# Q-Minh/point-cloud-processing

Measured on AMD Instinct MI355X. Metric: kNN+normal-estimation Mqueries/s (k=15), higher is better.
Workload: dtype f32

## Files before the change

### point-cloud-processing_amd/csrc/pcpx_api.hip

```cpp
#include "pcpx_internal.h"
#include "pcpx_radius.h"
#include "pcpx_features.h"

#include <algorithm>
#include <cstring>
#include <functional>
#include <vector>

namespace pcpx {
namespace {

struct Slice {
    u64 lo, hi, gf, gc;
};
Slice slice_of(const Index& ix, u64 sorted_first, u64 sorted_count)
{
    const u64 n = ix.n;
    Slice s;
    s.lo = sorted_first < n ? sorted_first : n;
    s.hi = sorted_count > n - s.lo ? n : s.lo + sorted_count;
    s.gf = s.lo / GROUP;
    const u64 gend = (s.hi + GROUP - 1) / GROUP;
    s.gc = gend > s.gf ? gend - s.gf : 0;
    return s;
// ... 878 lines not shown
    PCPX_HIP(hipMemcpy(dp.p, xyz, m * 3 * sizeof(float), hipMemcpyHostToDevice));
    if ((st = launch_normal_single(dp.as<float>(), m, dn.as<float>(), nullptr)) != PCPX_OK) return st;
    PCPX_HIP(hipMemcpy(out_normal, dn.p, 3 * sizeof(float), hipMemcpyDeviceToHost));
    return PCPX_OK;
    });
}

int pcpx_estimate_normals_batch(const float* xyz, const uint64_t* offsets, uint64_t nrows, int device, float* out_normals)
{
    return on_shared(device, "pcpx_estimate_normals_batch", [&](DeviceShared& shared) -> int {
    int st;
    if (nrows == 0) return PCPX_OK;
    if (!offsets || !out_normals) return PCPX_ERR_INVALID;
    for (u64 r = 0; r < nrows; ++r)
        if (offsets[r + 1] < offsets[r]) {
            set_error("pcpx_estimate_normals_batch: offsets must not decrease (row %llu)", static_cast<unsigned long long>(r));
            return PCPX_ERR_INVALID;
        }
    const u64 total = offsets[nrows] - offsets[0];
    if (total > 0 && !xyz) return PCPX_ERR_INVALID;
    DevBuf dp(shared.pool), doff(shared.pool), dn(shared.pool);
    if ((st = dp.alloc(total * 3 * sizeof(float))) != PCPX_OK || (st = doff.alloc((nrows + 1) * sizeof(u64))) != PCPX_OK ||
        (st = dn.alloc(nrows * 3 * sizeof(float))) != PCPX_OK)
        return st;
    if (total > 0) PCPX_HIP(hipMemcpyAsync(dp.p, xyz + 3 * offsets[0], total * 3 * sizeof(float), hipMemcpyHostToDevice, nullptr));
    PCPX_HIP(hipMemcpyAsync(doff.p, offsets, (nrows + 1) * sizeof(u64), hipMemcpyHostToDevice, nullptr));
    if ((st = launch_normals_csr(dp.as<float>(), doff.as<u64>(), nrows, dn.as<float>(), nullptr)) != PCPX_OK) return st;
    PCPX_HIP(hipMemcpyAsync(out_normals, dn.p, nrows * 3 * sizeof(float), hipMemcpyDeviceToHost, nullptr));
    PCPX_HIP(hipStreamSynchronize(nullptr));
    return PCPX_OK;
    });
}

int pcpx_debug_eps_test_mode(pcpx_index* h, int mode)
{
    return on_index(h, "pcpx_debug_eps_test_mode", ANY_INDEX, [&](Index* ix) -> int {
    if (mode < 0 || mode > 2) {
        set_error("pcpx_debug_eps_test_mode: mode is 0 (automatic), 1 (in the compaction) or 2 (per candidate)");
        return PCPX_ERR_INVALID;
    }
    ix->eps_test_mode = mode;
    return PCPX_OK;
    });
}

int pcpx_debug_set(pcpx_index* h, const char* name, int64_t value)
{
    return on_index(h, "pcpx_debug_set", ANY_INDEX, [&](Index* ix) -> int {
    if (!name) return PCPX_ERR_INVALID;
    const std::string key(name);
    if (key == "long_groups_first") {
        ix->tuning.lpt = value != 0;
        ix->sched.state = 0;
    } else if (key == "gather_outputs") {
        ix->tuning.gather = value != 0;
    } else if (key == "gather_counts") {
        ix->tuning.gather_counts = value != 0;
    } else {
        set_error("pcpx_debug_set: no setting called '%s'", name);
        return PCPX_ERR_INVALID;
    }
    return PCPX_OK;
    });
}

int pcpx_debug_get(pcpx_index* h, const char* name, int64_t* out_value)
{
    return on_index(h, "pcpx_debug_get", ANY_INDEX, [&](Index* ix) -> int {
    if (!name || !out_value) return PCPX_ERR_INVALID;
    const std::string key(name);
    if (key == "build_redos") {
        *out_value = ix->build_redos;
    } else if (key == "full_buckets") {
        int64_t c = 0;
        for (u32 w = 0; w < 8; ++w) c += __builtin_popcount(ix->full_buckets[w]);
        *out_value = c;
    } else if (key == "schedule_state") {
        *out_value = ix->sched.state;
    } else {
        set_error("pcpx_debug_get: no figure called '%s'", name);
        return PCPX_ERR_INVALID;
    }
    return PCPX_OK;
    });
}

int pcpx_debug_group_times(pcpx_index* h, uint32_t* out_ticks, uint64_t capacity, uint64_t* out_groups)
{
    return on_index(h, "pcpx_debug_group_times", ANY_INDEX, [&](Index* ix) -> int {
    if (!out_groups) return PCPX_ERR_INVALID;
    *out_groups = ix->sched.state ? ix->sched.gc : 0;
    if (*out_groups == 0) return PCPX_OK;
    if (!out_ticks || capacity < *out_groups) return PCPX_ERR_CAPACITY;
    PCPX_HIP(hipMemcpyAsync(out_ticks, ix->sched.d_gtime, *out_groups * sizeof(u32), hipMemcpyDeviceToHost, ix->stream));
    PCPX_HIP(hipStreamSynchronize(ix->stream));
    return PCPX_OK;
    });
}

int pcpx_knn_group_costs_dev(pcpx_index* h, uint32_t k, float eps, uint32_t group_stride, uint32_t* d_out_events, uint64_t capacity,
                             uint64_t* out_samples)
{
    return on_index(h, "pcpx_knn_group_costs_dev", ANY_INDEX, [&](Index* ix) -> int {
    if (!out_samples || group_stride == 0) return PCPX_ERR_INVALID;
    if (ix->shard.on) return shard_unsupported(*ix, "pcpx_knn_group_costs_dev");
    const u64 groups = (ix->n + GROUP - 1) / GROUP;
// ... 367 lines not shown
```

### point-cloud-processing_amd/csrc/pcpx_device.h

```cpp
#ifndef PCPX_DEVICE_H
#define PCPX_DEVICE_H

#include "pcpx_internal.h"

#include <cmath>
#include <limits>
#include <type_traits>

#pragma clang fp contract(off)

namespace pcpx {
namespace {

constexpr int WAVES_PER_BLOCK = 1;

__device__ __forceinline__ u32 wave_in_block() { return __builtin_amdgcn_readfirstlane(threadIdx.x >> 6); }

__device__ __forceinline__ u32 virtual_block()
{
    u32 per = gridDim.x >> 3;
    return (blockIdx.x & 7u) * per + (blockIdx.x >> 3);
}

__device__ __forceinline__ float sq3(float dx, float dy, float dz) { return dx * dx + dy * dy + dz * dz; }
// ... 25 lines not shown
    NodeBox4 out;
    u32* o = reinterpret_cast<u32*>(&out);
#pragma unroll
    for (int i = 0; i < 16; ++i) {
        o[i] = a[i];
        o[16 + i] = b[i];
    }
    return out;
}

__device__ __forceinline__ bool any_lane(bool c) { return __builtin_amdgcn_ballot_w64(c) != 0ull; }

template <class T>
__device__ __forceinline__ T load_const(const T* p)
{
    static_assert(sizeof(T) % 4 == 0, "record size");
    typedef const __attribute__((address_space(4))) u32* const_u32_ptr;
    const_u32_ptr c = (const_u32_ptr)(reinterpret_cast<uintptr_t>(p));
    T out;
    u32* o = reinterpret_cast<u32*>(&out);
#pragma unroll
    for (unsigned i = 0; i < sizeof(T) / 4; ++i) o[i] = c[i];
    return out;
}

__device__ __forceinline__ u32 lds_address(const void* p)
{
    return static_cast<u32>(reinterpret_cast<uintptr_t>(p));
}


template <bool X16, bool KEEP = false>
struct WalkerT {
    u64 pend;
    u32 ploc;
    int l;
    u64 leaf_need[W];

    static __device__ __forceinline__ u32 level_base(int d) { return 0x55555555u >> (32 - 2 * d); }

    template <class Need>
    __device__ __forceinline__ u32 child_mask(const TreeView& t, int d, u32 loc, Need&& need)
    {
        const u32 first_child = level_base(d + 1) + (loc << LOGW);
        const NodeBox4 cb = X16 ? load_node4(t.nodes + first_child) : load_const(reinterpret_cast<const NodeBox4*>(t.nodes + first_child));
        u32 m = 0;
#pragma unroll
        for (int c = W - 1; c >= 0; --c) {
            const u64 lanes = __builtin_amdgcn_ballot_w64(need(cb.c[c]));
            if (KEEP) leaf_need[c] = lanes;
            asm("s_cmp_lg_u64 %1, 0\n\ts_addc_u32 %0, %0, %0" : "+s"(m) : "s"(lanes) : "scc");
        }
        return m;
    }

    template <class Need>
    __device__ __forceinline__ bool start(const TreeView& t, Need&& need, u32& n_expand)
    {
        pend = 0;
        ploc = 0;
        l = 0;
        if (t.nleaves == 0) return false;
        const NodeBox root = load_const(t.nodes);
        if (!any_lane(need(root))) return false;
        if (t.depth == 0) return true;
        ++n_expand;
        l = t.depth - 1;
        pend = static_cast<u64>(child_mask(t, 0, 0u, need)) << (W * l);
        return false;
    }

    __device__ __forceinline__ bool done() const { return pend == 0; }
    __device__ __forceinline__ int pop(u32& loc)
    {
        int bit;
        asm("s_ff1_i32_b64 %0, %1\n\ts_bitset0_b64 %1, %0" : "=&s"(bit), "+s"(pend));
        const int h = bit >> LOGW;
        loc = ((ploc >> (LOGW * (h - l))) << LOGW) + (static_cast<u32>(bit) & (W - 1u));
        return h;
    }
    __device__ __forceinline__ void at_leaf(u32 loc)
    {
        ploc = loc >> LOGW;
        l = 0;
    }
    template <class Need>
    __device__ __forceinline__ void expand(const TreeView& t, int h, u32 loc, Need&& need)
    {
        l = h - 1;
        ploc = loc;
        pend |= static_cast<u64>(child_mask(t, t.depth - h, loc, need)) << (W * l);
    }

    template <class Need>
    __device__ __forceinline__ u32 leaves_of(const TreeView& t, u32 loc, Need&& need)
    {
        l = 0;
        ploc = loc;
        return child_mask(t, t.depth - 1, loc, need);
    }

    template <class Need>
    __device__ __forceinline__ bool next(const TreeView& t, Need&& need, u32& leaf, u32& n_expand)
    {
        while (pend != 0) {
            const int bit = __builtin_ctzll(pend);
// ... 76 lines not shown
```

### point-cloud-processing_amd/csrc/pcpx_internal.h

```cpp
#ifndef PCPX_INTERNAL_H
#define PCPX_INTERNAL_H

#include <cstring>
#include <hip/hip_runtime.h>

#include <cstdint>
#include <mutex>
#include <new>
#include <string>
#include <vector>

#include "pcpx.h"

namespace pcpx {

using u32 = std::uint32_t;
using u64 = std::uint64_t;

constexpr int LEAF = 8;
constexpr int LOGW = 2;
constexpr int W = 1 << LOGW;
constexpr int GROUP = 64;
constexpr int LEAVES_PER_GROUP = GROUP / LEAF;
constexpr int MAXDEPTH = 15;
// ... 118 lines not shown
    int idx_bits = 1;
    int sorted_from_bit = 24;
    const u64* finish_words = nullptr;
    const u32* finish_first_pass = nullptr;
    u32 full_buckets[8] = {0, 0, 0, 0, 0, 0, 0, 0};
    u32 build_redos = 0;
    u32 low_pass_tiles = ~0u;
    void* d_sort_tmp = nullptr;
    size_t sort_tmp_bytes = 0;
    Leaf* d_leaves = nullptr;
    NodeBox* d_nodes = nullptr;
    u64 nodes_cap = 0;
    u32* d_scalars = nullptr;
    u32 nleaves = 0;
    int depth = 0;
    u32 leaf0 = 0;

    struct Interval {
        int family;
        hipEvent_t a, b;
    };
    bool profiling = false;
    std::vector<Interval> intervals;

    u32* d_queue = nullptr;
    u32 queue_set = 0;
    u32* queue_now = nullptr;
    u32* queue_clear = nullptr;
    u64* d_multi = nullptr;
    size_t multi_bytes = 0;

    void* d_scratch = nullptr;
    size_t scratch_bytes = 0;

    hipStream_t copy_stream = nullptr;
    DevPool pool;
    PinnedStage pinned;
    u32 few_epoch = 0;
    struct Sched {
        u32* d_gtime = nullptr;
        u32* d_order = nullptr;
        u64 cap = 0;
        u64 gf = 0, gc = 0;
        int kcap = 0;
        u32 k = 0;
        int state = 0;
    } sched;
    float4* d_nc4 = nullptr;
    u32* d_pos_of = nullptr;
    u64 nc4_cap = 0, pos_of_cap = 0;
    bool pos_of_valid = false;
    struct Tuning {
        int lpt = 1;
        int gather_counts = 0;
        int gather = 0;
    } tuning;
    int eps_test_mode = 0;

    struct Shard {
        bool on = false;
        u32 rank = 0, world = 1;
        u64 n_glob = 0;
        u64 g_first = 0, g_count = 0;
        u64 core_g0 = 0;
        u64 core_l0 = 0;
        u64 core_count = 0;
        u32 halo_cells = 0;
        u32 k_hint = 0;
        bool explicit_range = false;
        u64 range_first = 0, range_count = 0;
        bool everything = false;
        bool borrowed = false;
        const float* cloud = nullptr;
        u32* d_sel = nullptr;
        u32* d_need = nullptr;
        u32* d_grid = nullptr;
        u32* d_hist12 = nullptr;
        u32* d_plan = nullptr;
        u32* d_big = nullptr;
        u32* d_tile_cnt = nullptr;
        u64 tile_cap = 0;
        u64* d_words = nullptr;
        float* d_tau = nullptr;
        u32* d_fail = nullptr;
        u64 cap_loc = 0;
        u32 verified_k = 0;
        float verified_eps = -1.f;
        u64 verified_first = 0, verified_count = 0;
        u64 last_failed = 0, total_failed = 0, enlargements = 0;
    } shard;

    const u64* sorted_codes() const { return finish_words ? finish_words : d_codes[1]; }
    u32* perm() const { return d_perm; }
    TreeView view() const { return TreeView{d_leaves, d_nodes, nleaves, static_cast<u32>(n), depth, leaf0}; }
};

struct ProfileScope {
    Index& ix;
    int family;
    hipEvent_t a = nullptr, b = nullptr;
    ProfileScope(Index& i, int fam) : ix(i), family(fam)
    {
        if (!ix.profiling) return;
        if (hipEventCreate(&a) != hipSuccess || hipEventCreate(&b) != hipSuccess) {
            a = b = nullptr;
            return;
// ... 297 lines not shown
```

### point-cloud-processing_amd/csrc/pcpx_query.hip

```cpp
#include "pcpx_device.h"
#include "pcpx_eig3.h"

namespace pcpx {

namespace {

constexpr size_t STATS_EXTRA = 16 + 5 * 65536 - 8;
constexpr u64 PAD_KEY = 0x7F800000FFFFFFFFull;

__device__ __forceinline__ u64 pad_key_here()
{
    u32 lo = static_cast<u32>(PAD_KEY), hi = static_cast<u32>(PAD_KEY >> 32);
    asm volatile("" : "+v"(lo), "+v"(hi));
    return (static_cast<u64>(hi) << 32) | lo;
}

__device__ __forceinline__ void ce(u64& a, u64& b)
{
    double x = __longlong_as_double(static_cast<long long>(a)), y = __longlong_as_double(static_cast<long long>(b));
    double lo, hi;
    asm("v_min_f64 %0, %1, %2" : "=v"(lo) : "v"(x), "v"(y));
    asm("v_max_f64 %0, %1, %2" : "=v"(hi) : "v"(x), "v"(y));
    a = static_cast<u64>(__double_as_longlong(lo));
    b = static_cast<u64>(__double_as_longlong(hi));
// ... 279 lines not shown
                 "v_add_u32_e32 %[pos], 1, %[pos]"
                 : [wa] "+v"(wa), [pos] "+v"(pos)
                 : [d2] "v"(d2), [tau] "v"(tau), [lo] "s"(lo), [sv] "s"(saved)
                 : "vcc", "memory");
}

__device__ __forceinline__ void append_if_shell(float d2, float tau, float lo, float dx, float dy, float dz, float eps, u32& pos,
                                                u32& wa, u64 saved)
{
    float m = fmaxf(fmaxf(fabsf(dx), fabsf(dy)), fabsf(dz));
    asm volatile("v_cmpx_le_f32_e32 %[d2], %[tau]\n\t"
                 "v_cmpx_lt_f32_e32 %[lo], %[d2]\n\t"
                 "v_cmpx_le_f32_e32 %[eps], %[m]\n\t"
                 "ds_write2_b32 %[wa], %[pos], %[d2] offset1:1\n\t"
                 "v_add_u32_e32 %[wa], 0x200, %[wa]\n\t"
                 "s_mov_b64 exec, %[sv]\n\t"
                 "v_add_u32_e32 %[pos], 1, %[pos]"
                 : [wa] "+v"(wa), [pos] "+v"(pos)
                 : [d2] "v"(d2), [tau] "v"(tau), [lo] "s"(lo), [m] "v"(m), [eps] "s"(eps), [sv] "s"(saved)
                 : "vcc", "memory");
}

constexpr int MINW8 = 8;
constexpr int MINW16 = 7;
constexpr int MINW32 = 4;
template <int KCAP>
constexpr float cap_mult() { return KCAP <= 8 ? 1.375f : KCAP <= 16 ? 1.25f : 1.125f; }
constexpr float CAP_GROW = 4.f;
template <int KCAP>
__device__ __forceinline__ float wave_radius_cap(float tau, bool valid, u32 lane)
{
    const float inf = std::numeric_limits<float>::infinity();
    asm volatile("" : "+v"(lane));
    const bool sample = (lane & 3u) == 1u;
    const float x = (valid && tau < inf) ? tau : inf;
    const u64 finite = __builtin_amdgcn_ballot_w64(sample && x < inf);
    const u32 nfinite = static_cast<u32>(__builtin_popcountll(finite));
    if (nfinite == 0) {
        const u64 any = __builtin_amdgcn_ballot_w64(x < inf);
        if (any == 0) return inf;
        return __uint_as_float(__builtin_amdgcn_readlane(__float_as_uint(x), static_cast<u32>(__builtin_ctzll(any)))) * cap_mult<KCAP>();
    }
    u32 rank = 0;
#pragma unroll
    for (u32 l = 1; l < 64; l += 4) {
        const float other = __uint_as_float(__builtin_amdgcn_readlane(__float_as_uint(x), l));
        rank += (other < x || (other == x && l < lane)) ? 1u : 0u;
    }
    const u64 is_med = __builtin_amdgcn_ballot_w64(sample && x < inf && rank == nfinite / 2);
    const float med = __uint_as_float(__builtin_amdgcn_readlane(__float_as_uint(x), static_cast<u32>(__builtin_ctzll(is_med))));
    return med * cap_mult<KCAP>();
}

struct MultiPass {
    const u64* lo = nullptr;
    u64* lo_out = nullptr;
    u64* keys = nullptr;
    u32 stride = 0;
    u32 offset = 0;
    u32 slot0 = 0;
};

struct KnnArgs {
    TreeView t;
    QueryView qv;
    u32 group_first, group_end, k;
    float eps, eps_thr;
    KnnOutputs o;
    MultiPass mp;
    u32* queue;
    unsigned long long* stats;
    KnnSchedule sch;
    u32* queue_clear;
};
typedef const __attribute__((address_space(4))) KnnArgs* knn_args_ptr;
__device__ __forceinline__ knn_args_ptr knn_args_here()
{
    u64 a = reinterpret_cast<u64>(__builtin_amdgcn_kernarg_segment_ptr());
    u32 lo = static_cast<u32>(a), hi = static_cast<u32>(a >> 32);
    asm volatile("" : "+s"(lo), "+s"(hi));
    return reinterpret_cast<knn_args_ptr>((static_cast<u64>(hi) << 32) | lo);
}
template <class T>
__device__ __forceinline__ T cold(const __attribute__((address_space(4))) T* field)
{
    static_assert(sizeof(T) % 4 == 0, "dwords");
    T out;
    u32* o = reinterpret_cast<u32*>(&out);
    const __attribute__((address_space(4))) u32* c = reinterpret_cast<const __attribute__((address_space(4))) u32*>(field);
#pragma unroll
    for (unsigned i = 0; i < sizeof(T) / 4; ++i) o[i] = c[i];
    return out;
}

template <int KCAP, bool SELF, int DIAG, bool MULTI, bool EPS_EACH, int NZ>
__device__ __forceinline__ void knn_group(const TreeView& tree, const u32 g, const float eps, const float eps_thr,
                                          unsigned long long* __restrict__ stats, u64* __restrict__ col, float* __restrict__ pub, const u32 lane,
                                          const u32 slot, const u32 part)
{
    constexpr bool STATS = DIAG == 1, COST = DIAG == 2;
    constexpr int BUF = buf_rows(KCAP);
    TreeView t = tree;
    asm volatile("" : "+s"(t.depth), "+s"(t.nodes));
    __builtin_amdgcn_s_setprio(PRIO_BASE);
    const knn_args_ptr ka = knn_args_here();
    const u32 k_arg = ka->k;
    const u32 pos_lo = ka->o.pos_lo, pos_hi = ka->o.pos_hi;
    MultiPass mp;
    if (MULTI) mp = cold(&ka->mp);
    const float* const known_d2 = STATS ? cold(&ka->o.d2) : nullptr;
    u32 k_here = k_arg;
    asm volatile("" : "+s"(k_here));
    const u32 k = k_here;
    u32 st_leaves = 0, st_expand = 0, st_compact = 0, st_app = 0, st_round2 = 0, st_seed_compact = 0, st_seed_app = 0, st_sparse = 0, st_owners = 0;
    u32 st_steps = 0;
    unsigned long long tc_walk = 0, tc_compact = 0, tc_leaf = 0, tc0 = 0, tc_mark = 0, tc_later_mark = 0;
    u32 st_later_lanes = 0;
    if (STATS) tc0 = __builtin_amdgcn_s_memtime();
    u32 tick0 = 0;
    if (!MULTI && DIAG == 0) tick0 = static_cast<u32>(__builtin_amdgcn_s_memtime());

    u32 p_here = g * GROUP + lane;
    asm volatile("" : "+v"(p_here));
    const u32 p = p_here;
    const u32 nq = SELF ? t.n : ka->qv.nq;
    const bool mine_of_part = ((p >> 3) & 7u) + 1u == part;
    const bool valid = p < nq && (!SELF || p - pos_lo < pos_hi - pos_lo) && (part == 0u || mine_of_part);
    float qx = 0.f, qy = 0.f, qz = 0.f;
    if (valid) {
        if (SELF) {
            const Leaf& lf = t.leaves[p / LEAF];
            qx = lf.x[p % LEAF];
            qy = lf.y[p % LEAF];
            qz = lf.z[p % LEAF];
        } else {
            qx = cold(&ka->qv.qx)[p];
            qy = cold(&ka->qv.qy)[p];
            qz = cold(&ka->qv.qz)[p];
        }
    }
    asm volatile("" : "+v"(qx), "+v"(qy), "+v"(qz));
    u64 lo_key = 0;
    bool has_lo = false;
    if (MULTI && mp.lo && valid) {
        lo_key = mp.lo[p - mp.slot0];
        has_lo = true;
    }
    u64 best[KCAP];
#pragma unroll
    for (int j = 0; j < KCAP; ++j) best[j] = (j < KCAP - static_cast<int>(k)) ? 0ull : PAD_KEY;
    const float inf = std::numeric_limits<float>::infinity();
    float tau = valid ? inf : -1.f;
    float tau_known = inf;
// ... 192 lines not shown
            u32 at, inside;
            if (packed_free > 0)
                asm volatile("v_cmpx_le_f32_e32 %[d2], %[tau]\n\t"
                             "v_mov_b32_e32 %[at], 0x200\n\t"
                             "ds_add_rtn_u32 %[at], %[slot], %[at]\n\t"
                             "s_waitcnt lgkmcnt(0)\n\t"
                             "v_subrev_u32_e32 %[m], %[end], %[at]\n\t"
                             "v_ashrrev_i32_e32 %[m], 31, %[m]\n\t"
                             "v_bfi_b32 %[at], %[m], %[at], %[spare]\n\t"
                             "ds_write2_b32 %[at], %[pos], %[d2] offset1:1\n\t"
                             "s_mov_b64 exec, %[saved]"
                             : [at] "=&v"(at), [m] "=&v"(inside)
                             : [d2] "v"(d2), [tau] "v"(q.w), [slot] "v"(slot), [end] "s"(wa_end), [spare] "s"(wa_end + 480u), [pos] "v"(posj), [saved] "s"(saved)
                             : "vcc", "memory");
            else
                asm volatile("v_cmpx_le_f32_e32 %[d2], %[tau]\n\t"
                             "v_mov_b32_e32 %[at], 0x200\n\t"
                             "ds_add_rtn_u32 %[at], %[slot], %[at]\n\t"
                             "s_waitcnt lgkmcnt(0)\n\t"
                             "ds_write2_b32 %[at], %[pos], %[d2] offset1:1\n\t"
                             "s_mov_b64 exec, %[saved]"
                             : [at] "=&v"(at)
                             : [d2] "v"(d2), [tau] "v"(q.w), [slot] "v"(slot), [pos] "v"(posj), [saved] "s"(saved)
                             : "vcc", "memory");
            s += 8u;
        } while (s < how_many);
        __builtin_amdgcn_wave_barrier();
        u32 now = wa;
        if (mine) {
            now = pub_wa[r];
            reinterpret_cast<float*>(pub_q + r)[3] = -1.f;
        }
        __builtin_amdgcn_wave_barrier();
        __builtin_amdgcn_s_setprio(PRIO_BASE);
        if (packed_free == 0) {
            wa = now;
            return 0ull;
        }
        const bool lost_keys = now > col_addr + (static_cast<u32>(BUF) << 9);
        wa = lost_keys ? wa : now;
        return __builtin_amdgcn_ballot_w64(lost_keys);
    };
    auto packed_take_back = [&](const u64 lost) {
        if (__builtin_amdgcn_inverse_ballot_w64(lost)) {
            const u32 column_end = col_addr + (static_cast<u32>(BUF) << 9);
            const u64 pad = pad_key_here();
            for (u32 a = wa; a < column_end; a += 512u) asm volatile("ds_write_b64 %0, %1" ::"v"(a), "v"(pad) : "memory");
        }
    };
    const u32 seed_count = s1 - s0;
    u32 packed_limit = packed_leaves ? PACKED_LEAVES : 0;
    for (u32 rounds = 0;;) {
        const u32 packed_limit_now = __builtin_amdgcn_readfirstlane(packed_limit);
        bool root_leaf = wk.start(t, need, st_expand);
        (void)root_leaf;
        if (STATS) tc_mark = __builtin_amdgcn_s_memtime();
        u32 direct = 0, direct_first = 0;
        for (;;) {
            if (direct == 0) {
                if (wk.done()) break;
                u32 node;
                const int h = wk.pop(node);
                ++st_expand;
                if (h > 1) {
                    wk.expand(t, h, node, need);
                } else {
                    direct_first = node << LOGW;
                    direct = wk.leaves_of(t, node, need);
                }
            }
            while (direct != 0) {
                u32 loc;
                {
                    u32 child;
                    asm("s_ff1_i32_b32 %0, %1\n\ts_bitset0_b32 %1, %0" : "=&s"(child), "+s"(direct));
                    loc = direct_first + child;
                }
                if (loc - s0 >= seed_count) {
                    if (STATS) tc_walk += __builtin_amdgcn_s_memtime() - tc_mark;
                    if (!packed_leaves) {
                        fold_if_needed(true, false);
                        candidates(loc, rounds != 0u);
                    } else {
                        const u32 c = loc & (W - 1u);
                        u64 who;
                        u32 how_many;
                        asm("s_cmp_eq_u32 %[c], 2\n\ts_cselect_b64 %[w], %[n2], %[n3]\n\t"
                            "s_cmp_eq_u32 %[c], 1\n\ts_cselect_b64 %[w], %[n1], %[w]\n\t"
                            "s_cmp_eq_u32 %[c], 0\n\ts_cselect_b64 %[w], %[n0], %[w]\n\t"
                            "s_bcnt1_i32_b64 %[m], %[w]"
                            : [w] "=&s"(who), [m] "=s"(how_many)
                            : [c] "s"(c), [n0] "s"(wk.leaf_need[0]), [n1] "s"(wk.leaf_need[1]), [n2] "s"(wk.leaf_need[2]), [n3] "s"(wk.leaf_need[3])
                            : "scc");
                        u32 packed_form, full_from;
                        asm("s_cmp_le_u32 %[m], %[lim]\n\ts_cselect_b32 %[pf], 1, 0\n\ts_cselect_b32 %[thr], %[tp], %[td]"
                            : [pf] "=&s"(packed_form), [thr] "=&s"(full_from)
                            : [m] "s"(how_many), [lim] "s"(packed_limit_now), [tp] "s"(wa_packed_full), [td] "s"(wa_full)
                            : "scc");
                        u64 todo = who;
                        for (;;) {
                            if ((__builtin_amdgcn_ballot_w64(wa >= full_from) & todo) != 0) fold(false);
                            if (packed_form == 0u) break;
                            if (STATS) tc_mark = __builtin_amdgcn_s_memtime();
                            todo = packed_leaf(loc, todo, how_many);
                            if (COST) st_steps += (how_many + 7u) >> 3;
                            if (STATS) {
                                asm volatile("" ::"v"(wa));
                                tc_leaf += __builtin_amdgcn_s_memtime() - tc_mark;
                            }
                            if (__builtin_expect(todo == 0, 1)) break;
                            packed_take_back(todo);
                            how_many = static_cast<u32>(__builtin_popcountll(todo));
                            full_from = 0u;
                        }
                        if (packed_form != 0u) {
                            if (COST) ++st_sparse;
                            if (STATS) ++st_leaves, ++st_sparse, st_owners += how_many;
// ... 103 lines not shown
        u32 id = t.leaves[ps / LEAF].id[ps % LEAF];
        asm volatile("" : "+v"(id));
        best[s] = real ? ((key & 0xFFFFFFFF00000000ull) | id) : key;
    }
    bool unordered = false;
#pragma unroll
    for (int s = 0; s + 1 < KCAP; ++s) unordered |= best[s] > best[s + 1];
    for (int round = 0; round < KCAP && any_lane(unordered); ++round) {
#pragma unroll
        for (int parity = 0; parity < 2; ++parity) {
#pragma unroll
            for (int s = parity; s + 1 < KCAP; s += 2) {
                const bool sw = best[s] > best[s + 1];
                const u64 a = sw ? best[s + 1] : best[s], b = sw ? best[s] : best[s + 1];
                best[s] = a;
                best[s + 1] = b;
                if (sw) {
                    const u32 pa = pos_slot(s), pb = pos_slot(s + 1);
                    pos_slot(s) = pb;
                    pos_slot(s + 1) = pa;
                }
            }
        }
        unordered = false;
#pragma unroll
        for (int s = 0; s + 1 < KCAP; ++s) unordered |= best[s] > best[s + 1];
    }
    auto restore_column = [&]() {
        const u64 pad = pad_key_here();
#pragma unroll
        for (int r = 0; r < (KCAP + 1) / 2; ++r) col[r * 64] = pad;
    };

    if (!valid) {
        restore_column();
        return;
    }
    u32 g_again = g;
    asm volatile("" : "+s"(g_again));
    u32 p_row = g_again * GROUP + lane;
    asm volatile("" : "+v"(p_row));
    const knn_args_ptr kb = knn_args_here();
    const KnnOutputs o = cold(&kb->o);
    u32 row = SELF ? t.leaves[p_row / LEAF].id[p_row % LEAF] : cold(&kb->qv.row)[p_row];
    if (SELF && o.by_position) row = p_row + o.pos_bias;
    if (SELF && o.tau) o.tau[p_row] = key_d2(best[KCAP - 1]);
    u32 found = 0;
    u32 okmask = 0;
    const u32 stride = o.row_stride ? o.row_stride : k;
    const u64 ob = static_cast<u64>(row) * stride;
    const bool whole_rows = stride == static_cast<u32>(KCAP) && first_slot == NZ && !STATS;
    auto store_whole_rows = [&](auto FS) {
        constexpr int fs = decltype(FS)::value;
#pragma unroll
        for (int c = 0; c < KCAP / 4; ++c) {
            u32 id4[4];
            float d4[4];
#pragma unroll
            for (int e = 0; e < 4; ++e) {
                const int sl = 4 * c + e + fs;
                const u64 key = sl < KCAP ? best[sl < KCAP ? sl : 0] : PAD_KEY;
                const bool ok = key != PAD_KEY;
                id4[e] = ok ? static_cast<u32>(key) : INVALID_ID;
                d4[e] = __uint_as_float(static_cast<u32>(key >> 32));
            }
            if (o.idx) *reinterpret_cast<uint4*>(o.idx + ob + 4 * c) = make_uint4(id4[0], id4[1], id4[2], id4[3]);
            if (o.d2) *reinterpret_cast<float4*>(o.d2 + ob + 4 * c) = make_float4(d4[0], d4[1], d4[2], d4[3]);
        }
    };
    if (whole_rows) store_whole_rows(std::integral_constant<int, NZ>{});
#pragma unroll
    for (int s = NZ; s < KCAP; ++s) {
        int j = s - first_slot;
        if (j >= 0) {
            u64 key = best[s];
            bool ok = key != PAD_KEY;
            if (!whole_rows) {
                if (o.idx) o.idx[ob + j] = ok ? static_cast<u32>(key) : INVALID_ID;
                if (o.d2 && !STATS) o.d2[ob + j] = __uint_as_float(static_cast<u32>(key >> 32));
            }
            found += ok ? 1u : 0u;
            okmask |= ok ? (1u << s) : 0u;
        }
    }
    if (!whole_rows) {
        for (u32 j = k; j < stride; ++j) {
            if (o.idx) o.idx[ob + j] = INVALID_ID;
            if (o.d2 && !STATS) o.d2[ob + j] = __uint_as_float(static_cast<u32>(PAD_KEY >> 32));
        }
    }
    if (o.cnt) o.cnt[row] = found;

    if (o.meandist) {
        float sum = 0.f;
#pragma unroll
        for (int s = NZ; s < KCAP; ++s) {
            bool ok = (okmask >> s) & 1u;
            float d = sqrtf(__uint_as_float(static_cast<u32>(best[s] >> 32)));
            sum += ok ? d : 0.f;
        }
        o.meandist[row] = sum / static_cast<float>(found);
    }

    if (o.normals || o.centroids || (SELF && o.nc4)) {
        float nbx[KCAP], nby[KCAP], nbz[KCAP];
#pragma unroll
        for (int s = NZ; s < KCAP; ++s) {
            const u32 ps = pos_slot(s);
            const Leaf& lf = t.leaves[ps / LEAF];
            nbx[s] = lf.x[ps % LEAF];
            nby[s] = lf.y[ps % LEAF];
            nbz[s] = lf.z[ps % LEAF];
        }
        float sx = 0.f, sy = 0.f, sz = 0.f;
#pragma unroll
        for (int s = NZ; s < KCAP; ++s) {
// ... 5 lines not shown
        float fn = static_cast<float>(found);
        float mx = sx / fn, my = sy / fn, mz = sz / fn;
        if (o.centroids) {
            o.centroids[3ull * row] = mx;
            o.centroids[3ull * row + 1] = my;
            o.centroids[3ull * row + 2] = mz;
        }
        if (!o.normals && !(SELF && o.nc4)) {
            restore_column();
            return;
        }
        float c00 = 0.f, c10 = 0.f, c11 = 0.f, c20 = 0.f, c21 = 0.f, c22 = 0.f;
#pragma unroll
        for (int s = NZ; s < KCAP; ++s) {
            bool ok = (okmask >> s) & 1u;
            float x = nbx[s], y = nby[s], z = nbz[s];
            float vx = ok ? x - mx : 0.f, vy = ok ? y - my : 0.f, vz = ok ? z - mz : 0.f;
            c00 += vx * vx;
            c10 += vy * vx;
            c11 += vy * vy;
            c20 += vz * vx;
            c21 += vz * vy;
            c22 += vz * vz;
        }
        float nrm[3], ev[3];
        eig3_smallest(c00, c10, c20, c11, c21, c22, nrm, ev);
        if (SELF && o.nc4) {
            o.nc4[p_row] = make_float4(nrm[0], nrm[1], nrm[2], __uint_as_float(found));
        } else {
            o.normals[3ull * row] = nrm[0];
            o.normals[3ull * row + 1] = nrm[1];
            o.normals[3ull * row + 2] = nrm[2];
        }
    }
    restore_column();
}

constexpr u32 QUEUE_STRIDE = 16;
constexpr u32 ORDER_HEADER = 16, ORDER_PARTS = 8, ORDER_PART_SHIFT = 28, ORDER_GROUP_MASK = (1u << ORDER_PART_SHIFT) - 1u;
inline u64 order_entries(u64 ngroups) { return ORDER_HEADER + ORDER_PARTS * 8ull * ((ngroups + 7) / 8); }

template <int KCAP, bool SELF, int DIAG, bool MULTI = false, bool EPS_EACH = false, int NZ = 0>
__global__ __launch_bounds__(64 * knn_wpb(KCAP, MULTI), KCAP <= 8 ? MINW8 : KCAP <= 16 ? MINW16 : MINW32) void k_knn(
    const KnnArgs a)
{
    constexpr bool STATS = DIAG == 1;
    const TreeView t = a.t;
    const float eps = a.eps, eps_thr = a.eps_thr;
    unsigned long long* const __restrict__ stats = STATS ? a.stats : nullptr;
    constexpr int BUF = buf_rows(KCAP);
    extern __shared__ u64 lds[];
    const u32 lane = threadIdx.x & 63u;
    const u32 wib = wave_in_block();
    u64* const rows = lds + static_cast<size_t>(wib) * lds_rows(BUF, MULTI, MULTI ? 0 : KCAP) * 64;
    u64* col = rows + lane;
    float* pub = reinterpret_cast<float*>(rows + BUF * 64);
    if (pack_rows(MULTI, KCAP) > 0 && lane < static_cast<u32>(PACKED_LEAVES)) pub[4u * lane + 3u] = -1.f;
    if (blockIdx.x == 0 && wib == 0 && lane < 8u) a.queue_clear[lane * QUEUE_STRIDE] = 0u;
    if (chunked_compaction(MULTI)) {
        const u64 pad = pad_key_here();
#pragma unroll
        for (int j = 0; j < BUF; ++j) col[j * 64] = pad;
    }
    unsigned long long t_start = 0, t_max = 0, g_max = 0;
    u32 n_done = 0;
    if (STATS) t_start = __builtin_amdgcn_s_memrealtime();
    for (u32 s = 0; s < 8u;) {
        const knn_args_ptr ka = knn_args_here();
        const u32 group_first = ka->group_first, group_end = ka->group_end;
        u32* const queue = cold(&ka->queue);
        const u32 ngroups = group_end - group_first;
        const u32 per = (ngroups + 7u) >> 3;
        const u32 q = (blockIdx.x + s) & 7u;
        const u32 qbeg = q * per;
        const u32 qend = qbeg + per < ngroups ? qbeg + per : ngroups;
        u32 gi = 0, lane_here = lane;
        asm volatile("" : "+v"(lane_here));
        if (lane_here == 0) gi = atomicAdd(&queue[q * QUEUE_STRIDE], 1u);
        gi = __builtin_amdgcn_readfirstlane(gi);
        const u32* const order = cold(&ka->sch.order);
        if (order ? gi >= load_const(order + q) : qbeg + gi >= qend) {
            ++s;
            continue;
        }
        unsigned long long tg = 0, tcg = 0;
        if (STATS) {
            tg = __builtin_amdgcn_s_memrealtime();
            tcg = __builtin_amdgcn_s_memtime();
        }
        const u32 entry = order ? load_const(order + ORDER_HEADER + ORDER_PARTS * qbeg + gi) : group_first + qbeg + gi;
        const u32 g = entry & ORDER_GROUP_MASK;
        knn_group<KCAP, SELF, DIAG, MULTI, EPS_EACH, NZ>(t, g, eps, eps_thr, stats, col, pub, lane, qbeg + gi, entry >> ORDER_PART_SHIFT);
        if (STATS) {
            if (lane == 0) atomicAdd(&stats[11], static_cast<unsigned long long>(__builtin_amdgcn_s_memtime()) - tcg);
            ++n_done;
            tg = __builtin_amdgcn_s_memrealtime() - tg;
            if (tg > t_max) {
                t_max = tg;
                g_max = g;
            }
        }
    }
    if (STATS && lane == 0 && wib == 0) {
        stats[16 + 5ull * blockIdx.x] = t_start;
        stats[17 + 5ull * blockIdx.x] = __builtin_amdgcn_s_memrealtime();
        stats[18 + 5ull * blockIdx.x] = n_done;
        stats[19 + 5ull * blockIdx.x] = t_max;
// ... 107 lines not shown
#pragma unroll
        for (u32 bb = 0; bb < 3; ++bb) {
            const u64 m = __builtin_amdgcn_ballot_w64(b == bb);
            if (lane == 0) wave_s[bb][w] = static_cast<u32>(__builtin_popcountll(m));
            if (b == bb) below = __builtin_amdgcn_mbcnt_hi(static_cast<u32>(m >> 32), __builtin_amdgcn_mbcnt_lo(static_cast<u32>(m), 0u));
        }
        __syncthreads();
        if (in) {
            u32 before = 0;
            for (u32 ww = 0; ww < w; ++ww) before += wave_s[b][ww];
            const u32 at = ORDER_HEADER + ORDER_PARTS * qbeg;
            if (b == 0) {
#pragma unroll
                for (u32 part = 0; part < ORDER_PARTS; ++part) order[at + ORDER_PARTS * (base_s[0] + before + below) + part] = (group_first + i) | ((part + 1u) << ORDER_PART_SHIFT);
            } else {
                order[at + (ORDER_PARTS - 1u) * cnt_s[0] + base_s[b] + before + below] = group_first + i;
            }
        }
        __syncthreads();
        if (t < 3) {
            u32 tot = 0;
            for (u32 ww = 0; ww < 16; ++ww) tot += wave_s[t][ww];
            base_s[t] += tot;
        }
        __syncthreads();
    }
}

int sched_reserve(Index& ix, u64 groups)
{
    Index::Sched& sc = ix.sched;
    if (groups <= sc.cap) return PCPX_OK;
    PCPX_HIP(hipStreamSynchronize(ix.stream));
    index_block_free(sc.d_gtime);
    index_block_free(sc.d_order);
    sc = Index::Sched{};
    const u64 cap = groups + groups / 8 + 64;
    void *a = nullptr, *b = nullptr;
    if (index_block_alloc(&a, cap * sizeof(u32)) != hipSuccess || index_block_alloc(&b, order_entries(cap) * sizeof(u32)) != hipSuccess) {
        (void)hipGetLastError();
        index_block_free(a);
        index_block_free(b);
        return PCPX_ERR_ALLOC;
    }
    sc.d_gtime = static_cast<u32*>(a);
    sc.d_order = static_cast<u32*>(b);
    sc.cap = cap;
    return PCPX_OK;
}

template <int KCAP, bool SELF, bool EPS_EACH, int NZ>
static int launch_knn_form(Index& ix, const QueryView& qv, u64 gfirst, u64 gcount, u32 k, float eps, float thr, const KnnOutputs& o)
{
    constexpr int BUF = buf_rows(KCAP);
    constexpr int WPB = knn_wpb(KCAP, false);
    const size_t lds = static_cast<size_t>(WPB) * lds_rows(BUF, false, KCAP) * 64 * sizeof(u64);
    const u32 gf = static_cast<u32>(gfirst), ge = static_cast<u32>(gfirst + gcount);
    if (o.row_stride != 0 && (o.row_stride < k || ((o.row_stride == static_cast<u32>(KCAP)) && ((reinterpret_cast<uintptr_t>(o.idx) | reinterpret_cast<uintptr_t>(o.d2)) & 15u) != 0))) {
        set_error("pcpx: row_stride must be >= k, and rows of %d entries must start at multiples of 16 bytes", KCAP);
        return PCPX_ERR_INVALID;
    }
    int st = prepare_queue(ix);
    if (st != PCPX_OK) return st;
    KnnSchedule sch;
    auto* fn = k_knn<KCAP, SELF, 0, false, EPS_EACH, NZ>;
    const u32 pgrid = persistent_grid(ix, reinterpret_cast<const void*>(fn), 64 * WPB, lds, gcount, WPB);
    if (SELF && ix.tuning.lpt && gcount >= LPT_MIN_GROUPS) {
        Index::Sched& sc = ix.sched;
        const bool same = sc.state != 0 && sc.gf == gfirst && sc.gc == gcount && sc.kcap == KCAP && sc.k == k;
        if (same && sc.state == 1) {
            k_make_order<<<8, 1024, 0, ix.stream>>>(sc.d_gtime, static_cast<u32>(gcount), gf, sc.d_order);
            sc.state = 2;
        }
        if (same && sc.state == 2) {
            sch.order = sc.d_order;
        } else if (sched_reserve(ix, gcount) == PCPX_OK) {
            sch.gtime = sc.d_gtime;
            sc.gf = gfirst, sc.gc = gcount, sc.kcap = KCAP, sc.k = k, sc.state = 1;
        }
    }
    ProfileScope prof(ix, PCPX_K_KNN);
    fn<<<pgrid, 64 * WPB, lds, ix.stream>>>(KnnArgs{ix.view(), qv, gf, ge, k, eps, thr, o, MultiPass{}, ix.queue_now, nullptr, sch, ix.queue_clear});
    return check_hip(hipGetLastError(), "k_knn launch", __FILE__, __LINE__);
}

__global__ void k_sample_order(u32 nsamples, u32 stride, u32* __restrict__ order)
{
    const u32 i = blockIdx.x * blockDim.x + threadIdx.x;
    const u32 per = (nsamples + 7u) >> 3;
    if (i < 8u) {
        const u32 qbeg = i * per, qend = qbeg + per < nsamples ? qbeg + per : nsamples;
        order[i] = qend > qbeg ? qend - qbeg : 0u;
    }
    if (i < nsamples) order[ORDER_HEADER + ORDER_PARTS * (i / per * per) + i % per] = i * stride + stride / 2u;
}
template <int KCAP, int NZ>
static int launch_knn_cost_form(Index& ix, u32 nsamples, u32 k, float eps, float thr, const u32* d_order, u32* d_events)
{
    constexpr int BUF = buf_rows(KCAP);
    constexpr int WPB = knn_wpb(KCAP, false);
    const size_t lds = static_cast<size_t>(WPB) * lds_rows(BUF, false, KCAP) * 64 * sizeof(u64);
    int st = prepare_queue(ix);
    if (st != PCPX_OK) return st;
    auto* fn = k_knn<KCAP, true, 2, false, false, NZ>;
    const u32 pgrid = persistent_grid(ix, reinterpret_cast<const void*>(fn), 64 * WPB, lds, nsamples, WPB);
    QueryView qv{nullptr, nullptr, nullptr, nullptr, nullptr, static_cast<u32>(ix.n)};
    KnnSchedule sch;
    sch.order = d_order;
    sch.events = d_events;
    fn<<<pgrid, 64 * WPB, lds, ix.stream>>>(KnnArgs{ix.view(), qv, 0u, nsamples, k, eps, thr, KnnOutputs{}, MultiPass{}, ix.queue_now, nullptr, sch, ix.queue_clear});
    return check_hip(hipGetLastError(), "k_knn cost sample launch", __FILE__, __LINE__);
}

template <int KCAP>
static int launch_knn_t(Index& ix, const QueryView& qv, bool self, u64 gfirst, u64 gcount, u32 k, float eps, const KnnOutputs& o)
{
    const float thr = eps_box_threshold(ix, eps);
    if (thr >= 0.f) {
        if (k < static_cast<u32>(KCAP)) {
            return self ? launch_knn_form<KCAP, true, false, 1>(ix, qv, gfirst, gcount, k, eps, thr, o)
                        : launch_knn_form<KCAP, false, false, 1>(ix, qv, gfirst, gcount, k, eps, thr, o);
        }
        return self ? launch_knn_form<KCAP, true, false, 0>(ix, qv, gfirst, gcount, k, eps, thr, o)
                    : launch_knn_form<KCAP, false, false, 0>(ix, qv, gfirst, gcount, k, eps, thr, o);
    }
    return self ? launch_knn_form<KCAP, true, true, 0>(ix, qv, gfirst, gcount, k, eps, thr, o)
                : launch_knn_form<KCAP, false, true, 0>(ix, qv, gfirst, gcount, k, eps, thr, o);
}

template <bool SELF>
__global__ __launch_bounds__(256) void k_assemble(TreeView t, QueryView qv, u32 slot0, u32 nslots, u32 k, u32 stride,
                                                  u64* __restrict__ keys, KnnOutputs o)
{
    const u32 i = blockIdx.x * blockDim.x + threadIdx.x;
    if (i >= nslots) return;
// ... 201 lines not shown
```

Baseline: 2816.

## Test upper tree levels against one wave-wide search box in kNN traversal

Adds a mode for the k=16 kNN kernel where, once every lane holds a finite search radius, the wave computes one conservative axis-aligned box that covers all lanes' search balls. It reduces the coordinates with DPP and readlane, pads each bound outward by one ulp, and writes the box to LDS. At tree levels from depth 3 upward, child masks come from a single per-lane global load compared against that box via two ballots, in place of per-lane box-distance tests on scalar-loaded node boxes. This is meant to cut scalar loads and per-lane ALU work on high levels. The cost is a looser pruning test that may expand more nodes, plus a little extra LDS per wave.

Measured after the change: 2799. No clear change (-0.6%).

```diff
diff --git a/point-cloud-processing_amd/csrc/pcpx_api.hip b/point-cloud-processing_amd/csrc/pcpx_api.hip
--- a/point-cloud-processing_amd/csrc/pcpx_api.hip
+++ b/point-cloud-processing_amd/csrc/pcpx_api.hip
@@ -954,6 +954,8 @@
     if (key == "long_groups_first") {
         ix->tuning.lpt = value != 0;
         ix->sched.state = 0;
+    } else if (key == "knn_wave_levels") {
+        ix->tuning.wave_levels = value != 0;
     } else if (key == "gather_outputs") {
         ix->tuning.gather = value != 0;
     } else if (key == "gather_counts") {
diff --git a/point-cloud-processing_amd/csrc/pcpx_device.h b/point-cloud-processing_amd/csrc/pcpx_device.h
--- a/point-cloud-processing_amd/csrc/pcpx_device.h
+++ b/point-cloud-processing_amd/csrc/pcpx_device.h
@@ -101,6 +101,50 @@
             asm("s_cmp_lg_u64 %1, 0\n\ts_addc_u32 %0, %0, %0" : "+s"(m) : "s"(lanes) : "scc");
         }
         return m;
+    }
+
+    template <int BOX_AT>
+    __device__ __forceinline__ u32 child_mask_wave(const TreeView& t, int d, u32 loc, u32 row0, u32 lane)
+    {
+        const u32 first_child = level_base(d + 1) + (loc << LOGW);
+        const u64 address = reinterpret_cast<uintptr_t>(t.nodes + first_child);
+        const u32 address_lo = __builtin_amdgcn_readfirstlane(static_cast<u32>(address));
+        const u32 address_hi = __builtin_amdgcn_readfirstlane(static_cast<u32>(address >> 32));
+        const u64 uniform = (static_cast<u64>(address_hi) << 32) | address_lo;
+        asm volatile("" : "+v"(lane));
+        const u32 word = (lane & 31u) << 2;
+        const u32 mine = row0 | (word & 28u);
+        float v, b;
+        asm volatile("global_load_dword %0, %2, %3\n\tds_read_b32 %1, %4 offset:%5\n\ts_waitcnt vmcnt(0) lgkmcnt(0)"
+                     : "=&v"(v), "=&v"(b)
+                     : "v"(word), "s"(uniform), "v"(mine), "n"(BOX_AT));
+        const u32 le = static_cast<u32>(__builtin_amdgcn_ballot_w64(v <= b));
+        const u32 ge = static_cast<u32>(__builtin_amdgcn_ballot_w64(v >= b));
+        u32 m = (le & 0x47474747u) | (ge & 0x38383838u) | 0x80808080u;
+        m &= m >> 4;
+        m &= m >> 2;
+        m &= m >> 1;
+        return (((m & 0x01010101u) * 0x00204081u) >> 21) & 0xFu;
+    }
+    template <int BOX_AT, class Need>
+    __device__ __forceinline__ void start_wave(const TreeView& t, Need&& need, u32& n_expand, u32 row0, u32 lane)
+    {
+        pend = 0;
+        ploc = 0;
+        l = 0;
+        if (t.nleaves == 0) return;
+        const NodeBox root = load_const(t.nodes);
+        if (!any_lane(need(root))) return;
+        ++n_expand;
+        l = t.depth - 1;
+        pend = static_cast<u64>(child_mask_wave<BOX_AT>(t, 0, 0u, row0, lane)) << (W * l);
+    }
+    template <int BOX_AT>
+    __device__ __forceinline__ void expand_wave(const TreeView& t, int h, u32 loc, u32 row0, u32 lane)
+    {
+        l = h - 1;
+        ploc = loc;
+        pend |= static_cast<u64>(child_mask_wave<BOX_AT>(t, t.depth - h, loc, row0, lane)) << (W * l);
     }
 
     template <class Need>
diff --git a/point-cloud-processing_amd/csrc/pcpx_internal.h b/point-cloud-processing_amd/csrc/pcpx_internal.h
--- a/point-cloud-processing_amd/csrc/pcpx_internal.h
+++ b/point-cloud-processing_amd/csrc/pcpx_internal.h
@@ -194,6 +194,7 @@
     bool pos_of_valid = false;
     struct Tuning {
         int lpt = 1;
+        int wave_levels = 1;
         int gather_counts = 0;
         int gather = 0;
     } tuning;
diff --git a/point-cloud-processing_amd/csrc/pcpx_query.hip b/point-cloud-processing_amd/csrc/pcpx_query.hip
--- a/point-cloud-processing_amd/csrc/pcpx_query.hip
+++ b/point-cloud-processing_amd/csrc/pcpx_query.hip
@@ -355,6 +355,48 @@
     return med * cap_mult<KCAP>();
 }
 
+constexpr int WAVE_LEVELS_FROM = 3;
+__host__ __device__ constexpr bool wave_levels(int kcap, bool multi, int diag) { return !multi && diag == 0 && kcap == 16; }
+constexpr u32 WAVE_BOX_BYTES = 32;
+__host__ __device__ constexpr size_t knn_wave_lds(int kcap, bool multi, int diag)
+{
+    return static_cast<size_t>(lds_rows(buf_rows(kcap), multi, multi ? 0 : kcap)) * 64 * sizeof(u64) + (wave_levels(kcap, multi, diag) ? WAVE_BOX_BYTES : 0u);
+}
+__device__ __forceinline__ float one_ulp_outward(float x, bool up)
+{
+    const u32 bits = __float_as_uint(x);
+    const float stepped = __uint_as_float((x > 0.f) == up ? bits + 1u : bits - 1u);
+    const float from_zero = up ? std::numeric_limits<float>::min() : -std::numeric_limits<float>::min();
+    return (fabsf(x) < std::numeric_limits<float>::infinity()) ? (x == 0.f ? from_zero : stepped) : x;
+}
+__device__ __forceinline__ void wave_search_box(float qx, float qy, float qz, bool active, float cap, u32 box_row, u32 lane)
+{
+    const float inf = std::numeric_limits<float>::infinity();
+    float R = sqrtf(cap);
+    while (R * R < cap) R = one_ulp_outward(R, true);
+    R = one_ulp_outward(fmaxf(R, 0x1p-60f), true);
+    asm volatile("" : "+v"(lane));
+    const u32 j = lane & 7u;
+    float word = 0.f;
+#pragma unroll
+    for (u32 a = 0; a < 6u; ++a) {
+        const bool up = a < 3u;
+        const float q = a % 3u == 0u ? qx : a % 3u == 1u ? qy : qz;
+        float r = active ? q : (up ? -inf : inf);
+        auto other = [&](float x, float y) { return up ? fmaxf(x, y) : fminf(x, y); };
+        r = other(r, __int_as_float(__builtin_amdgcn_update_dpp(__float_as_int(r), __float_as_int(r), 0xB1, 0xF, 0xF, false)));
+        r = other(r, __int_as_float(__builtin_amdgcn_update_dpp(__float_as_int(r), __float_as_int(r), 0x4E, 0xF, 0xF, false)));
+        r = other(r, __int_as_float(__builtin_amdgcn_update_dpp(__float_as_int(r), __float_as_int(r), 0x141, 0xF, 0xF, false)));
+        r = other(r, __int_as_float(__builtin_amdgcn_update_dpp(__float_as_int(r), __float_as_int(r), 0x140, 0xF, 0xF, false)));
+        r = other(other(__uint_as_float(__builtin_amdgcn_readlane(__float_as_uint(r), 0)), __uint_as_float(__builtin_amdgcn_readlane(__float_as_uint(r), 16))),
+                  other(__uint_as_float(__builtin_amdgcn_readlane(__float_as_uint(r), 32)), __uint_as_float(__builtin_amdgcn_readlane(__float_as_uint(r), 48))));
+        r = one_ulp_outward(up ? r + R : r - R, up);
+        word = j == a ? r : word;
+        asm volatile("" : "+v"(word));
+    }
+    asm volatile("ds_write_b32 %0, %1" ::"v"(box_row + 4u * j), "v"(word) : "memory");
+}
+
 struct MultiPass {
     const u64* lo = nullptr;
     u64* lo_out = nullptr;
@@ -375,6 +417,7 @@
     unsigned long long* stats;
     KnnSchedule sch;
     u32* queue_clear;
+    u32 wave_levels;
 };
 typedef const __attribute__((address_space(4))) KnnArgs* knn_args_ptr;
 __device__ __forceinline__ knn_args_ptr knn_args_here()
@@ -402,6 +445,8 @@
                                           const u32 slot, const u32 part)
 {
     constexpr bool STATS = DIAG == 1, COST = DIAG == 2;
+    constexpr bool WAVE = wave_levels(KCAP, MULTI, DIAG);
+    constexpr int BOX_AT = lds_rows(buf_rows(KCAP), MULTI, MULTI ? 0 : KCAP) * 512;
     constexpr int BUF = buf_rows(KCAP);
     TreeView t = tree;
     asm volatile("" : "+s"(t.depth), "+s"(t.nodes));
@@ -700,8 +745,20 @@
     u32 packed_limit = packed_leaves ? PACKED_LEAVES : 0;
     for (u32 rounds = 0;;) {
         const u32 packed_limit_now = __builtin_amdgcn_readfirstlane(packed_limit);
-        bool root_leaf = wk.start(t, need, st_expand);
-        (void)root_leaf;
+        u32 wave_from = 0x7FFFFFFFu;
+        if (WAVE) {
+            const u32 capped = __builtin_amdgcn_readfirstlane(cap < inf ? 1u : 0u);
+            if (capped != 0u && knn_args_here()->wave_levels != 0u) {
+                wave_search_box(qx, qy, qz, active, cap, lds_row0 + BOX_AT, lane);
+                wave_from = WAVE_LEVELS_FROM;
+            }
+        }
+        if (WAVE && static_cast<u32>(t.depth) >= wave_from) {
+            wk.template start_wave<BOX_AT>(t, need, st_expand, lds_row0, lane);
+        } else {
+            bool root_leaf = wk.start(t, need, st_expand);
+            (void)root_leaf;
+        }
         if (STATS) tc_mark = __builtin_amdgcn_s_memtime();
         u32 direct = 0, direct_first = 0;
         for (;;) {
@@ -710,7 +767,9 @@
                 u32 node;
                 const int h = wk.pop(node);
                 ++st_expand;
-                if (h > 1) {
+                if (WAVE && static_cast<u32>(h) >= wave_from) {
+                    wk.template expand_wave<BOX_AT>(t, h, node, lds_row0, lane);
+                } else if (h > 1) {
                     wk.expand(t, h, node, need);
                 } else {
                     direct_first = node << LOGW;
@@ -920,6 +979,8 @@
     const bool whole_rows = stride == static_cast<u32>(KCAP) && first_slot == NZ && !STATS;
     auto store_whole_rows = [&](auto FS) {
         constexpr int fs = decltype(FS)::value;
+        u32 none = INVALID_ID;
+        asm volatile("" : "+v"(none));
 #pragma unroll
         for (int c = 0; c < KCAP / 4; ++c) {
             u32 id4[4];
@@ -929,7 +990,7 @@
                 const int sl = 4 * c + e + fs;
                 const u64 key = sl < KCAP ? best[sl < KCAP ? sl : 0] : PAD_KEY;
                 const bool ok = key != PAD_KEY;
-                id4[e] = ok ? static_cast<u32>(key) : INVALID_ID;
+                id4[e] = ok ? static_cast<u32>(key) : none;
                 d4[e] = __uint_as_float(static_cast<u32>(key >> 32));
             }
             if (o.idx) *reinterpret_cast<uint4*>(o.idx + ob + 4 * c) = make_uint4(id4[0], id4[1], id4[2], id4[3]);
@@ -1041,7 +1102,7 @@
     extern __shared__ u64 lds[];
     const u32 lane = threadIdx.x & 63u;
     const u32 wib = wave_in_block();
-    u64* const rows = lds + static_cast<size_t>(wib) * lds_rows(BUF, MULTI, MULTI ? 0 : KCAP) * 64;
+    u64* const rows = lds + static_cast<size_t>(wib) * (knn_wave_lds(KCAP, MULTI, DIAG) / sizeof(u64));
     u64* col = rows + lane;
     float* pub = reinterpret_cast<float*>(rows + BUF * 64);
     if (pack_rows(MULTI, KCAP) > 0 && lane < static_cast<u32>(PACKED_LEAVES)) pub[4u * lane + 3u] = -1.f;
@@ -1255,9 +1316,8 @@
 template <int KCAP, bool SELF, bool EPS_EACH, int NZ>
 static int launch_knn_form(Index& ix, const QueryView& qv, u64 gfirst, u64 gcount, u32 k, float eps, float thr, const KnnOutputs& o)
 {
-    constexpr int BUF = buf_rows(KCAP);
     constexpr int WPB = knn_wpb(KCAP, false);
-    const size_t lds = static_cast<size_t>(WPB) * lds_rows(BUF, false, KCAP) * 64 * sizeof(u64);
+    const size_t lds = static_cast<size_t>(WPB) * knn_wave_lds(KCAP, false, 0);
     const u32 gf = static_cast<u32>(gfirst), ge = static_cast<u32>(gfirst + gcount);
     if (o.row_stride != 0 && (o.row_stride < k || ((o.row_stride == static_cast<u32>(KCAP)) && ((reinterpret_cast<uintptr_t>(o.idx) | reinterpret_cast<uintptr_t>(o.d2)) & 15u) != 0))) {
         set_error("pcpx: row_stride must be >= k, and rows of %d entries must start at multiples of 16 bytes", KCAP);
@@ -1283,7 +1343,7 @@
         }
     }
     ProfileScope prof(ix, PCPX_K_KNN);
-    fn<<<pgrid, 64 * WPB, lds, ix.stream>>>(KnnArgs{ix.view(), qv, gf, ge, k, eps, thr, o, MultiPass{}, ix.queue_now, nullptr, sch, ix.queue_clear});
+    fn<<<pgrid, 64 * WPB, lds, ix.stream>>>(KnnArgs{ix.view(), qv, gf, ge, k, eps, thr, o, MultiPass{}, ix.queue_now, nullptr, sch, ix.queue_clear, static_cast<u32>(ix.tuning.wave_levels)});
     return check_hip(hipGetLastError(), "k_knn launch", __FILE__, __LINE__);
 }
 
```
